# voletiv/mcvd-pytorch

Hardware: NVIDIA H100
Metric: frames/sec @100 DDPM steps, SMMNIST 64x64 (higher is better)
Workload: dtype f32 (fp16 hi/lo split on wgmma, fp32 accumulate)

## Files before the change

mcvd_b200/csrc/conv_umma.cu:

```cuda
#include <cuda.h>
#include <cuda_fp16.h>

#include <algorithm>
#include <cstring>

#include "mcvd_common.cuh"
#include "umma_ptx.cuh"

namespace mcvd {

constexpr int MT = 128;

namespace {

using namespace ptx;

constexpr int NPROD = 96;
constexpr int W_LOAD = 3;
constexpr int W_CONS = 4;
constexpr int NTHREADS = 384;
constexpr float STAT_SCALE = 65536.0f;
constexpr int TAB_NB = 8;
constexpr int HP_MAX = 512;
constexpr int PPT = (HP_MAX + NPROD - 1) / NPROD;
constexpr int RAW_STAGES = 2;
constexpr int MAX_RESIDENT = 12;

struct ConvMaps {
  CUtensorMap src[4];
  CUtensorMap tab;
};

struct ConvArgs {
  const float* s0;
  const float* s1;
  const float* s2;
  const float* s3;
  int C2, C3, nKB0;
  const __half* wpk;
  const float* bias;
  const float* res;
  const float* tab;
  int tab_planar;
  float* dst;
  unsigned long long* stats;
  int NJ;
  int B, H, W, C0, C1, Cout;
  int ks;
  int Wp, Pimg;
  int Qtot;
  int KB;
  int HP;
  int boxn, nbox;
  int raw_off, raw_stage, tab_off;
  int RA;
  int halo0;
  int nKB;
  int NB;
  int SA;
  int NPI;
  int tiles_n, ntiles;
  int act_in, act_out;
  int split;
  int tab_nb;
  float wscale, oscale;
};

__device__ __forceinline__ int decode_pos(const ConvArgs& a, int q, int& b_out) {
  if (q < 0 || q >= a.Qtot) return -1;
  const int b = q / a.Pimg;
  const int r = q - b * a.Pimg;
  const int rr = r / a.Wp, cc = r - rr * a.Wp;
  b_out = b;
  if (a.ks == 3) {
    if (rr == 0 || cc == 0) return -1;
    return (b * a.H + (rr - 1)) * a.W + (cc - 1);
  }
  return (b * a.H + rr) * a.W + cc;
}

__device__ __forceinline__ int first_raw(const ConvArgs& a, int q) {
  q = max(q, 0);
  if (q >= a.Qtot) return a.B * a.H * a.W;
  if (a.ks == 1) return q;
  const int b = q / a.Pimg;
  const int r = q - b * a.Pimg;
  const int rr = r / a.Wp, cc = r - rr * a.Wp;
  if (rr == 0) return b * a.H * a.W;
  return (b * a.H + (rr - 1)) * a.W + (cc == 0 ? 0 : cc - 1);
}

template <int NT>
__global__ void __launch_bounds__(NTHREADS, 1) k_conv_umma(const ConvArgs a, const __grid_constant__ ConvMaps maps) {
  extern __shared__ __align__(1024) uint8_t smem_raw[];
  const int chunks = a.KB / 8;
  const uint32_t a_half_bytes = (uint32_t)chunks * a.HP * 16;
  const uint32_t a_stage_bytes = 2 * a_half_bytes;
  constexpr uint32_t b_step_bytes = 64u * NT;
  const uint32_t b_stage_bytes = (uint32_t)(a.KB / 16) * b_step_bytes;
  uint8_t* a_base = smem_raw;
  uint8_t* b_base = a_base + (size_t)a.SA * a_stage_bytes;
  uint8_t* raw_base = smem_raw + a.raw_off;
  int* pinfo = reinterpret_cast<int*>(raw_base + (size_t)a.RA * a.raw_stage);
  unsigned long long* stat_s = reinterpret_cast<unsigned long long*>(pinfo + PPT * NPROD);
  uint64_t* bars = reinterpret_cast<uint64_t*>(stat_s + (a.stats ? a.NJ * 2 * NT : 0));
  const uint32_t bar0 = smem_u32(bars);
  auto A_FULL = [&](int i) { return bar0 + 8u * i; };
  auto A_EMPTY = [&](int i) { return bar0 + 8u * (a.SA + i); };
  auto B_FULL = [&](int i) { return bar0 + 8u * (2 * a.SA + i); };
  auto B_EMPTY = [&](int i) { return bar0 + 8u * (2 * a.SA + a.NB + i); };
  auto R_FULL = [&](int i) { return bar0 + 8u * (2 * a.SA + 2 * a.NB + i); };
  const int groups_n = a.tiles_n / a.NPI;

  const int tid = threadIdx.x, warp = tid >> 5, lane = tid & 31;
  const int taps = a.ks * a.ks;

  if (tid == 0) {
    for (int i = 0; i < a.SA; ++i) { mbar_init(A_FULL(i), NPROD); mbar_init(A_EMPTY(i), 8); }
    for (int i = 0; i < a.NB; ++i) { mbar_init(B_FULL(i), 1); mbar_init(B_EMPTY(i), 8); }
    for (int i = 0; i < a.RA; ++i) mbar_init(R_FULL(i), 1);
    fence_barrier_init();
  }
  if (a.stats)
    for (int i = tid; i < a.NJ * 2 * NT; i += NTHREADS) stat_s[i] = 0ull;
  __syncthreads();

  if (warp < W_LOAD) {
    const bool has_tab = a.tab != nullptr;
    const uint32_t rowb = (uint32_t)a.KB * 4, smask = a.KB == 32 ? 7u : 3u;
    auto tile_b0_of = [&](int t) {
      const int q_first = (t / groups_n) * MT - a.halo0;
      return q_first <= 0 ? 0 : min(a.B - 1, q_first / a.Pimg);
    };
    const uint32_t raw0 = smem_u32(raw_base);
    const uint32_t main_bytes = (uint32_t)a.nbox * a.boxn * rowb, ctr_bytes = (uint32_t)MT * rowb;
    const uint32_t tab_bytes = (uint32_t)a.tab_nb * a.KB * (a.tab_planar ? 12 : 16);
    int it = blockIdx.x, ikb = 0, ig = 0;
    auto issue_next = [&]() {
      if (it >= a.ntiles) return;
      const int p0 = (it / groups_n) * MT;
      const bool seg2 = ikb >= a.nKB0;
      int si, cc0;
      if (!seg2) {
        const int c0 = ikb * a.KB;
        if (c0 < a.C0) { si = 0; cc0 = c0; } else { si = 1; cc0 = c0 - a.C0; }
      } else {
        const int c0 = (ikb - a.nKB0) * a.KB;
        if (c0 < a.C2) { si = 2; cc0 = c0; } else { si = 3; cc0 = c0 - a.C2; }
      }
      const bool use_tab = has_tab && !seg2;
      const uint32_t dst = raw0 + (uint32_t)(ig % a.RA) * a.raw_stage;
      const uint32_t bar = R_FULL(ig % a.RA);
      mbar_arrive_expect_tx(bar, (seg2 ? ctr_bytes : main_bytes) + (use_tab ? tab_bytes : 0u));
      if (seg2) {
        tma_load_2d(dst, &maps.src[si], cc0, first_raw(a, p0), bar);
      } else {
        const int r0 = first_raw(a, p0 - a.halo0);
        for (int i = 0; i < a.nbox; ++i)
          tma_load_2d(dst + (uint32_t)i * a.boxn * rowb, &maps.src[si], cc0, r0 + i * a.boxn, bar);
      }
      if (use_tab) {
        if (a.tab_planar) tma_load_3d(dst + a.tab_off, &maps.tab, ikb * a.KB, 0, tile_b0_of(it), bar);
        else tma_load_2d(dst + a.tab_off, &maps.tab, 4 * ikb * a.KB, tile_b0_of(it), bar);
      }
      ++ig;
      if (++ikb == a.nKB) { ikb = 0; it += gridDim.x; }
    };
    if (tid == 0)
      for (int i = 0; i < a.RA - 1; ++i) issue_next();
    int g = 0;
    for (int t = blockIdx.x; t < a.ntiles; t += gridDim.x) {
      const int p0 = (t / groups_n) * MT;
      const int tb0 = tile_b0_of(t);
      const int raw_m = first_raw(a, p0 - a.halo0), raw_c = first_raw(a, p0);
      for (int h = tid; h < a.HP; h += NPROD) {
        int b = tb0;
        const int pix = decode_pos(a, p0 - a.halo0 + h, b);
        pinfo[h] = pix < 0 ? -1 : ((b - tb0) << 16) | (pix - raw_m);
      }
      for (int kb = 0; kb < a.nKB; ++kb, ++g) {
        const int st = g % a.SA;
        const bool seg2 = kb >= a.nKB0;
        const bool use_tab = has_tab && !seg2;
        const int h_lo = seg2 ? a.halo0 : 0, h_hi = seg2 ? a.halo0 + MT : a.HP;
        const int roff = seg2 ? raw_c - raw_m : 0;
        named_bar_sync(1, NPROD);
        if (tid == 0) issue_next();
        mbar_wait(A_EMPTY(st), ((g / a.SA) & 1) ^ 1);
        const int rs = g % a.RA;
        mbar_wait(R_FULL(rs), (g / a.RA) & 1);
        const uint8_t* raw = raw_base + (size_t)rs * a.raw_stage;
        const float* tsm = reinterpret_cast<const float*>(raw + a.tab_off);
        uint8_t* hi_base = a_base + (size_t)st * a_stage_bytes;
        uint8_t* lo_base = hi_base + a_half_bytes;
        const int h0 = h_lo + (tid - h_lo % NPROD + NPROD) % NPROD;
#pragma unroll 1
        for (int h = h0; h < h_hi; h += NPROD) {
          const int info = pinfo[h];
          const bool pad = info < 0;
          const int bidx = info >> 16;
          const uint32_t row = (uint32_t)((info & 0xffff) - roff);
          float4 rv[8];
#pragma unroll
          for (int j = 0; j < 8; ++j)
            if (j < 2 * chunks) {
              const uint32_t off = row * rowb + 16u * j;
              rv[j] = pad ? make_float4(0.f, 0.f, 0.f, 0.f)
                          : *reinterpret_cast<const float4*>(raw + (off ^ (((off >> 7) & smask) << 4)));
            }
#pragma unroll
          for (int ch = 0; ch < 4; ++ch) {
            if (ch < chunks) {
              uint4 hv = make_uint4(0u, 0u, 0u, 0u), lv = hv;
              if (!pad) {
                float v[8] = {rv[2 * ch].x, rv[2 * ch].y, rv[2 * ch].z, rv[2 * ch].w,
                              rv[2 * ch + 1].x, rv[2 * ch + 1].y, rv[2 * ch + 1].z, rv[2 * ch + 1].w};
                if (use_tab) {
                  if (a.tab_planar) {
                    const float* tb = tsm + bidx * 3 * a.KB + ch * 8;
#pragma unroll
                    for (int e = 0; e < 8; ++e) v[e] = fmaf(v[e] - tb[e], tb[a.KB + e], tb[2 * a.KB + e]);
                  } else {
                    const float4* tb = reinterpret_cast<const float4*>(tsm) + bidx * a.KB + ch * 8;
#pragma unroll
                    for (int e = 0; e < 8; ++e) {
                      const float4 tv = tb[e];
                      v[e] = fmaf(v[e] - tv.x, tv.y * tv.z, tv.w);
                    }
                  }
                  if (a.act_in) silu_fast8(v);
                }
                uint32_t hw[4], lw[4];
#pragma unroll
                for (int e = 0; e < 4; ++e) split2(v[2 * e], v[2 * e + 1], hw[e], lw[e]);
                hv = make_uint4(hw[0], hw[1], hw[2], hw[3]);
                lv = make_uint4(lw[0], lw[1], lw[2], lw[3]);
              }
              const size_t off = ((size_t)ch * a.HP + h) * 16;
              *reinterpret_cast<uint4*>(hi_base + off) = hv;
              *reinterpret_cast<uint4*>(lo_base + off) = lv;
            }
          }
        }
        fence_proxy_async();
        mbar_arrive(A_FULL(st));
      }
    }
  } else if (warp == W_LOAD) {
    if (elect_one()) {
      const uint32_t b0 = smem_u32(b_base);
      const int per_tile = a.nKB0 * taps + (a.nKB - a.nKB0);
      int st = 0, ph = 1;
      for (int t = blockIdx.x; t < a.ntiles; t += gridDim.x)
       for (int j = 0; j < a.NPI; ++j) {
        const int nt = (t % groups_n) * a.NPI + j;
        const uint8_t* wsrc = reinterpret_cast<const uint8_t*>(a.wpk) + (size_t)nt * per_tile * b_stage_bytes;
        for (int i = 0; i < per_tile; ++i) {
          mbar_wait(B_EMPTY(st), ph);
          mbar_arrive_expect_tx(B_FULL(st), b_stage_bytes);
          bulk_g2s(b0 + (uint32_t)st * b_stage_bytes, wsrc + (size_t)i * b_stage_bytes, b_stage_bytes, B_FULL(st));
          if (++st == a.NB) { st = 0; ph ^= 1; }
        }
      }
    }
    __syncwarp();
  } else {
    const int wg = (warp - W_CONS) >> 2;
    const int wq = (warp - W_CONS) & 3;
    const int ksteps = a.KB / 16;
    const uint32_t a_lbo = (uint32_t)a.HP * 16;
    const uint64_t a_proto = make_desc(0, a_lbo, 128), b_proto = make_desc(0, NT * 16, 128);
    const uint32_t a_half16 = a_half_bytes >> 4, b_lo16 = 2u * NT;
    const uint32_t a0_16 = smem_u32(a_base) >> 4, b0_16 = smem_u32(b_base) >> 4;
    const uint32_t a_stage16 = a_stage_bytes >> 4, b_stage16 = b_stage_bytes >> 4;
    const uint32_t a_lbo16 = a_lbo >> 4;
    int bst = 0, bph = 0, g0 = 0;
    for (int t = blockIdx.x; t < a.ntiles; t += gridDim.x, g0 += a.nKB)
     for (int j = 0; j < a.NPI; ++j) {
      const int p0 = (t / groups_n) * MT;
      const int n0 = ((t % groups_n) * a.NPI + j) * NT;
      const bool last_n = j == a.NPI - 1;
      float acc[NT / 2];
#pragma unroll
      for (int i = 0; i < NT / 2; ++i) acc[i] = 0.f;
      int pend_b = -1, pend_a = -1;
      for (int kb = 0; kb < a.nKB; ++kb) {
        const int g = g0 + kb;
        const int st = g % a.SA;
        mbar_wait(A_FULL(st), (g / a.SA) & 1);
        const uint32_t a_hi16 = a0_16 + (uint32_t)st * a_stage16 + (uint32_t)(a.halo0 + 64 * wg);
        const int ntap = (kb < a.nKB0) ? taps : 1;
        for (int tap = 0; tap < ntap; ++tap) {
          mbar_wait(B_FULL(bst), bph);
          const int shift = (a.ks == 3 && kb < a.nKB0) ? ((tap / 3 - 1) * a.Wp + (tap % 3 - 1)) : 0;
          const uint32_t a_tap16 = a_hi16 + (uint32_t)shift;
          const uint32_t b_tap16 = b0_16 + (uint32_t)bst * b_stage16;
          wgmma_fence();
#pragma unroll 1
          for (int s = 0; s < ksteps; ++s) {
            const uint64_t dbh = desc_add(b_proto, b_tap16 + (uint32_t)s * (b_step_bytes >> 4));
            const uint64_t dbl = desc_add(dbh, b_lo16);
            const uint64_t dah = desc_add(a_proto, a_tap16 + (uint32_t)(2 * s) * a_lbo16);
            const uint64_t dal = desc_add(dah, a_half16);
            wgmma_ss<NT>(acc, dah, dbh, 1);
            if (a.split & 1) wgmma_ss<NT>(acc, dal, dbh, 1);
            if (a.split & 2) wgmma_ss<NT>(acc, dah, dbl, 1);
          }
          wgmma_commit();
          wgmma_wait<1>();
          if (pend_b >= 0 && lane == 0) mbar_arrive(B_EMPTY(pend_b));
          if (pend_a >= 0 && lane == 0) mbar_arrive(A_EMPTY(pend_a));
          pend_b = bst;
          pend_a = (tap == ntap - 1 && last_n) ? st : -1;
          if (++bst == a.NB) { bst = 0; bph ^= 1; }
        }
      }
      wgmma_wait<0>();
#pragma unroll
      for (int i = 0; i < NT / 2; ++i) reg_fence(acc[i]);
      if (lane == 0) { mbar_arrive(B_EMPTY(pend_b)); if (pend_a >= 0) mbar_arrive(A_EMPTY(pend_a)); }

      const int r0 = 64 * wg + 16 * wq + (lane >> 2);
      const int cq = 2 * (lane & 3);
      int pix[2], slot[2];
      const int tile_b0 = min(a.B - 1, p0 / a.Pimg);
#pragma unroll
      for (int i = 0; i < 2; ++i) {
        int b = 0;
        pix[i] = decode_pos(a, p0 + r0 + 8 * i, b);
        slot[i] = pix[i] >= 0 ? b - tile_b0 : -1;
      }
      unsigned jmask = 0;
      if (a.stats) {
#pragma unroll 1
        for (int jj = 0; jj < a.NJ; ++jj)
          if (__ballot_sync(0xffffffffu, slot[0] == jj || slot[1] == jj)) jmask |= 1u << jj;
      }
#pragma unroll
      for (int j = 0; j < NT / 8; ++j) {
        const int n = n0 + 8 * j + cq;
        const float2 bv = a.bias ? __ldg(reinterpret_cast<const float2*>(a.bias + n)) : make_float2(0.f, 0.f);
        float v[2][2];
#pragma unroll
        for (int i = 0; i < 2; ++i) {
          float2 rv = make_float2(0.f, 0.f);
          if (a.res && pix[i] >= 0) rv = __ldg(reinterpret_cast<const float2*>(a.res + (long long)pix[i] * a.Cout + n));
          float x0 = (acc[4 * j + 2 * i] * a.wscale + bv.x + rv.x) * a.oscale;
          float x1 = (acc[4 * j + 2 * i + 1] * a.wscale + bv.y + rv.y) * a.oscale;
          if (a.act_out) { x0 = silu_f(x0); x1 = silu_f(x1); }
          v[i][0] = x0; v[i][1] = x1;
          if (pix[i] >= 0) *reinterpret_cast<float2*>(a.dst + (long long)pix[i] * a.Cout + n) = make_float2(x0, x1);
        }
        if (a.stats) {
#pragma unroll 1
          for (int jj = 0; jj < a.NJ; ++jj) {
            if (!(jmask & (1u << jj))) continue;
#pragma unroll
            for (int e = 0; e < 2; ++e) {
              long long s1 = 0;
              unsigned long long s2 = 0;
#pragma unroll
              for (int i = 0; i < 2; ++i) {
                if (slot[i] == jj) {
                  const int xi = __float2int_rn(v[i][e] * STAT_SCALE);
                  s1 += xi;
                  s2 += (unsigned long long)((long long)xi * (long long)xi);
                }
              }
#pragma unroll
              for (int o = 4; o <= 16; o <<= 1) {
                s1 += __shfl_xor_sync(0xffffffffu, s1, o);
                s2 += __shfl_xor_sync(0xffffffffu, s2, o);
              }
              if (lane < 4) {
                unsigned long long* sp = stat_s + (size_t)jj * 2 * NT + 8 * j + cq + e;
                atomicAdd(sp, (unsigned long long)s1);
                atomicAdd(sp + NT, s2);
              }
            }
          }
        }
      }
      if (a.stats) {
        named_bar_sync(2, 256);
        const int et = tid - W_CONS * 32;
        unsigned long long* gp = a.stats + (size_t)(p0 / MT) * a.NJ * 2 * a.Cout;
        for (int i = et; i < a.NJ * 2 * NT; i += 256) {
          const int jp = i / NT, n = i - jp * NT;
          gp[(size_t)jp * a.Cout + n0 + n] = stat_s[i];
          stat_s[i] = 0ull;
        }
        named_bar_sync(2, 256);
      }
    }
  }
}

__global__ void k_pack_weights(const float* __restrict__ w, __half* __restrict__ out, int taps, int Cin, int Cout,
                               int NT, int KB, float scale, int stage_off, int per_unit) {
  const int ksteps = KB / 16, nKB = Cin / KB, nNT = Cout / NT;
  const long long total = (long long)nNT * nKB * taps * ksteps * 2 * NT * 8;
  for (long long i = (long long)blockIdx.x * blockDim.x + threadIdx.x; i < total;
       i += (long long)gridDim.x * blockDim.x) {
    int e = (int)(i % 8);
    long long t = i / 8;
    int n = (int)(t % NT); t /= NT;
    int j = (int)(t % 2); t /= 2;
    int s = (int)(t % ksteps); t /= ksteps;
    int tap = (int)(t % taps); t /= taps;
    int kb = (int)(t % nKB); t /= nKB;
    int nt = (int)t;
    int c = kb * KB + s * 16 + j * 8 + e;
    float v = w[((long long)tap * Cin + c) * Cout + nt * NT + n] * scale;
    __half h = __float2half_rn(v);
    __half l = __float2half_rn(v - __half2float(h));
    long long step = ((long long)nt * per_unit + stage_off + (long long)kb * taps + tap) * ksteps + s;
    long long base = step * (4LL * NT * 8);
    long long o = (long long)(j * NT + n) * 8 + e;
    out[base + o] = h;
    out[base + 2LL * NT * 8 + o] = l;
  }
}

int pick_kb(int C0, int C1) {
  if (C0 % 32 == 0 && C1 % 32 == 0) return 32;
  if (C0 % 16 == 0 && C1 % 16 == 0) return 16;
  return 0;
}

int conv_kb(int C0, int C1, int C2, int C3) {
  int kb = pick_kb(C0, C1);
  if (C2 + C3 > 0 && pick_kb(C2, C3) < kb) kb = pick_kb(C2, C3);
  return kb;
}

struct Plan {
  int HP, NB, NJ;
  int boxn, nbox, tab_nb;
  int raw_off, raw_stage, tab_off, RA;
  size_t smem;
};

constexpr size_t SMEM_LIMIT = 227 * 1024;

size_t round1024(size_t x) { return (x + 1023) & ~(size_t)1023; }

bool make_plan(int H, int W, int ks, int KB, int NT, bool stats, int SA, Plan& p) {
  const int Wp = ks == 3 ? W + 1 : W;
  const int Pimg = ks == 3 ? (H + 1) * (W + 1) : H * W;
  const int halo0 = ks == 3 ? Wp + 1 : 0;
  p.HP = (MT + 2 * halo0 + 7) & ~7;
  p.NJ = (MT - 1) / Pimg + 2;
  if (p.HP > HP_MAX) return false;
  p.nbox = p.HP > 256 ? 2 : 1;
  p.boxn = p.nbox == 1 ? p.HP : ((p.HP / 2 + 7) & ~7);
  p.tab_nb = std::min(p.HP / Pimg + 2, TAB_NB);
  p.tab_off = p.nbox * p.boxn * KB * 4;
  p.raw_stage = (int)round1024((size_t)p.tab_off + (size_t)p.tab_nb * KB * 16);
  const size_t a_stage = (size_t)2 * (KB / 8) * p.HP * 16;
  const size_t b_stage = (size_t)(KB / 16) * 64 * NT;
  const size_t stat_bytes = stats ? (size_t)p.NJ * 2 * NT * 8 : 0;
  const size_t pinfo_bytes = (size_t)PPT * NPROD * 4;
  size_t bar_bytes = 0, fixed = 0;
  for (p.RA = RAW_STAGES; p.RA >= 1; --p.RA) {
    bar_bytes = 8 * (2 * SA + 20 + p.RA);
    fixed = round1024(SA * a_stage) + (size_t)p.RA * p.raw_stage + pinfo_bytes + stat_bytes + bar_bytes;
    if (fixed + 2 * b_stage <= SMEM_LIMIT) break;
  }
  if (p.RA == 0) return false;
  p.NB = (int)((SMEM_LIMIT - fixed) / b_stage);
  if (p.NB > 10) p.NB = 10;
  p.raw_off = (int)round1024(SA * a_stage + (size_t)p.NB * b_stage);
  p.smem = (size_t)p.raw_off + (size_t)p.RA * p.raw_stage + pinfo_bytes + stat_bytes + bar_bytes;
  return p.smem <= SMEM_LIMIT;
}

using EncodeTiled = CUresult (*)(CUtensorMap*, CUtensorMapDataType, cuuint32_t, void*, const cuuint64_t*,
                                 const cuuint64_t*, const cuuint32_t*, const cuuint32_t*, CUtensorMapInterleave,
                                 CUtensorMapSwizzle, CUtensorMapL2promotion, CUtensorMapFloatOOBfill);

EncodeTiled encode_tiled() {
  static const EncodeTiled fn = [] {
    void* f = nullptr;
    cudaDriverEntryPointQueryResult q;
    if (cudaGetDriverEntryPoint("cuTensorMapEncodeTiled", &f, cudaEnableDefault, &q) != cudaSuccess ||
        q != cudaDriverEntryPointSuccess)
      f = nullptr;
    return reinterpret_cast<EncodeTiled>(f);
  }();
  return fn;
}

int encode_map(CUtensorMap* m, const float* base, int rank, const cuuint64_t* dims, const cuuint64_t* strides,
               const cuuint32_t* box, CUtensorMapSwizzle swz, const char* name) {
  MCVD_CHECK(((uintptr_t)base & 15) == 0, "%s: TMA source %p is not 16-byte aligned", name, (const void*)base);
  for (int i = 0; i < rank; ++i)
    MCVD_CHECK(box[i] >= 1 && box[i] <= 256, "%s: TMA box dimension %u outside [1, 256]", name, box[i]);
  for (int i = 0; i < rank - 1; ++i)
    MCVD_CHECK(strides[i] % 16 == 0, "%s: TMA stride %llu bytes is not a multiple of 16", name,
               (unsigned long long)strides[i]);
  const EncodeTiled enc = encode_tiled();
  MCVD_CHECK(enc != nullptr, "%s: cuTensorMapEncodeTiled unavailable", name);
  const cuuint32_t estr[3] = {1, 1, 1};
  const CUresult r = enc(m, CU_TENSOR_MAP_DATA_TYPE_FLOAT32, (cuuint32_t)rank, const_cast<float*>(base), dims, strides,
                         box, estr, CU_TENSOR_MAP_INTERLEAVE_NONE, swz, CU_TENSOR_MAP_L2_PROMOTION_L2_128B,
                         CU_TENSOR_MAP_FLOAT_OOB_FILL_NONE);
  MCVD_CHECK(r == CUDA_SUCCESS, "%s: cuTensorMapEncodeTiled failed (%d)", name, (int)r);
  return 0;
}

template <int NT>
int launch_nt(const ConvArgs& a, const ConvMaps& m, size_t smem, int grid, cudaStream_t s) {
  cudaError_t e = cudaFuncSetAttribute(k_conv_umma<NT>, cudaFuncAttributeMaxDynamicSharedMemorySize, (int)smem);
  MCVD_CHECK(e == cudaSuccess, "CONV_UMMA: cudaFuncSetAttribute failed: %s", cudaGetErrorString(e));
  k_conv_umma<NT><<<grid, NTHREADS, smem, s>>>(a, m);
  MCVD_CUDA_LAUNCH_CHECK("conv_umma");
  return 0;
}

int launch_conv(const McvdOp& op, cudaStream_t s, bool planar) {
  const char* name = planar ? "CONV_UMMA2" : "CONV_UMMA";
  MCVD_CHECK(op.src0 && op.w && op.dst && (op.C1 == 0 || op.src1), "%s: null pointer", name);
  MCVD_CHECK(op.i0 == 1 || op.i0 == 3, "%s: kernel size %d unsupported", name, op.i0);
  ConvArgs a;
  a.s0 = (const float*)op.src0; a.s1 = (const float*)op.src1; a.wpk = (const __half*)op.w;
  a.s2 = (const float*)op.src2; a.s3 = (const float*)op.src3; a.C2 = op.src2 ? op.C2 : 0; a.C3 = op.src3 ? op.C3 : 0;
  a.bias = (const float*)op.bias; a.res = (const float*)op.aux0; a.tab = (const float*)op.aux1;
  a.tab_planar = planar ? 1 : 0;
  a.dst = (float*)op.dst;
  a.stats = (unsigned long long*)op.dst2;
  a.B = op.B; a.H = op.H; a.W = op.W; a.C0 = op.C0; a.C1 = op.C1; a.Cout = op.Cout; a.ks = op.i0;
  const int NT = op.i1;
  a.KB = conv_kb(op.C0, op.C1, a.C2, a.C3);
  MCVD_CHECK(a.KB != 0, "%s: input channels (%d,%d | %d,%d) must be multiples of 16", name, op.C0, op.C1, a.C2, a.C3);
  MCVD_CHECK(!planar || op.i2 == 0 || op.i2 == a.KB, "CONV_UMMA2: weights packed for K-block %d, the conv uses %d",
             op.i2, a.KB);
  MCVD_CHECK(NT >= 16 && NT <= 256 && NT % 16 == 0 && op.Cout % NT == 0, "%s: n tile %d invalid for Cout %d", name, NT,
             op.Cout);
  if (a.ks == 3) { a.Wp = op.W + 1; a.Pimg = (op.H + 1) * (op.W + 1); }
  else { a.Wp = op.W; a.Pimg = op.H * op.W; }
  MCVD_CHECK((long long)op.B * a.Pimg < (1LL << 31), "%s: too many pixels", name);
  a.Qtot = op.B * a.Pimg;
  MCVD_CHECK(!a.stats || a.Pimg >= 64, "%s: epilogue statistics need images of >= 64 positions", name);
  a.halo0 = (a.ks == 3) ? a.Wp + 1 : 0;
  a.nKB0 = (op.C0 + op.C1) / a.KB;
  a.nKB = a.nKB0 + (a.C2 + a.C3) / a.KB;
  a.tiles_n = op.Cout / NT;
  long long tiles_m = (a.Qtot + MT - 1) / MT;
  if (planar) tiles_m = (tiles_m + 1) & ~1LL;
  int dev = 0, sms = 132;
  cudaGetDevice(&dev);
  cudaDeviceGetAttribute(&sms, cudaDevAttrMultiProcessorCount, dev);
  const int mode = planar ? 0 : op.i2;
  MCVD_CHECK(mode >= 0 && mode <= 2, "%s: work organisation %d", name, mode);
  Plan p;
  const bool can_stay = a.ks == 1 && a.nKB == a.nKB0 && a.tiles_n > 1 && a.nKB <= MAX_RESIDENT &&
                        make_plan(op.H, op.W, a.ks, a.KB, NT, a.stats != nullptr, a.nKB, p);
  const bool stay = can_stay && (mode == 2 || (mode == 0 && 2 * tiles_m >= sms));
  a.SA = stay ? a.nKB : 2;
  a.NPI = stay ? a.tiles_n : 1;
  MCVD_CHECK(make_plan(op.H, op.W, a.ks, a.KB, NT, a.stats != nullptr, a.SA, p),
             "%s: tile does not fit shared memory (W=%d)", name, op.W);
  a.HP = p.HP; a.NB = p.NB; a.NJ = p.NJ;
  a.boxn = p.boxn; a.nbox = p.nbox; a.raw_off = p.raw_off; a.raw_stage = p.raw_stage; a.tab_off = p.tab_off;
  a.RA = p.RA;
  a.act_in = (op.flags & MCVD_F_ACT_IN) ? 1 : 0;
  a.act_out = (op.flags & MCVD_F_ACT_OUT) ? 1 : 0;
  a.wscale = op.f1; a.oscale = op.f0;
  a.split = (op.i3 >= 1 && op.i3 <= 3) ? op.i3 : (op.i3 == 4 ? 0 : 3);
  {
    const int nb = a.HP / a.Pimg + 2;
    MCVD_CHECK(nb <= TAB_NB || !a.tab, "%s: %dx%d images are too small for the fused-norm path", name, op.H, op.W);
    a.tab_nb = (nb <= TAB_NB) ? nb : 0;
  }
  ConvMaps maps;
  memset(&maps, 0, sizeof(maps));
  {
    const float* srcs[4] = {a.s0, a.s1, a.s2, a.s3};
    const int cs[4] = {a.C0, a.C1, a.C2, a.C3};
    const CUtensorMapSwizzle swz = a.KB == 32 ? CU_TENSOR_MAP_SWIZZLE_128B : CU_TENSOR_MAP_SWIZZLE_64B;
    for (int i = 0; i < 4; ++i) {
      if (!cs[i]) continue;
      MCVD_CHECK(srcs[i] != nullptr, "%s: null source %d", name, i);
      const cuuint64_t dims[2] = {(cuuint64_t)cs[i], (cuuint64_t)op.B * op.H * op.W};
      const cuuint64_t strides[1] = {(cuuint64_t)cs[i] * 4};
      const cuuint32_t box[2] = {(cuuint32_t)a.KB, (cuuint32_t)(i < 2 ? a.boxn : MT)};
      if (encode_map(&maps.src[i], srcs[i], 2, dims, strides, box, swz, name)) return -1;
    }
    if (a.tab) {
      const int Cin = op.C0 + op.C1;
      if (planar) {
        const cuuint64_t dims[3] = {(cuuint64_t)Cin, 3, (cuuint64_t)op.B};
        const cuuint64_t strides[2] = {(cuuint64_t)Cin * 4, (cuuint64_t)Cin * 12};
        const cuuint32_t box[3] = {(cuuint32_t)a.KB, 3, (cuuint32_t)a.tab_nb};
        if (encode_map(&maps.tab, a.tab, 3, dims, strides, box, CU_TENSOR_MAP_SWIZZLE_NONE, name)) return -1;
      } else {
        const cuuint64_t dims[2] = {(cuuint64_t)Cin * 4, (cuuint64_t)op.B};
        const cuuint64_t strides[1] = {(cuuint64_t)Cin * 16};
        const cuuint32_t box[2] = {(cuuint32_t)(4 * a.KB), (cuuint32_t)a.tab_nb};
        if (encode_map(&maps.tab, a.tab, 2, dims, strides, box, CU_TENSOR_MAP_SWIZZLE_NONE, name)) return -1;
      }
    }
  }
  MCVD_CHECK(tiles_m * a.tiles_n < (1LL << 31), "%s: too many tiles", name);
  a.ntiles = (int)(tiles_m * (a.tiles_n / a.NPI));
  const int grid = a.ntiles < sms ? a.ntiles : sms;
  switch (NT) {
#define MCVD_NT_CASE(n) case n: return launch_nt<n>(a, maps, p.smem, grid, s);
    MCVD_NT_CASE(16) MCVD_NT_CASE(32) MCVD_NT_CASE(48) MCVD_NT_CASE(64) MCVD_NT_CASE(80) MCVD_NT_CASE(96)
    MCVD_NT_CASE(112) MCVD_NT_CASE(128) MCVD_NT_CASE(144) MCVD_NT_CASE(160) MCVD_NT_CASE(176) MCVD_NT_CASE(192)
    MCVD_NT_CASE(208) MCVD_NT_CASE(224) MCVD_NT_CASE(240) MCVD_NT_CASE(256)
#undef MCVD_NT_CASE
    default: break;
  }
  MCVD_CHECK(false, "%s: n tile %d", name, NT);
}

long long pack(const float* w_taps, int taps, int Cin, int Cout, int n_tile, int KB, void* out, int scale_log2,
               int stage_off, int per_unit, void* stream) {
  if ((KB != 16 && KB != 32) || Cin % KB || n_tile < 16 || n_tile % 16 || Cout % n_tile) {
    set_error("umma_pack_weights: Cin %d / Cout %d / n_tile %d / KB %d unsupported", Cin, Cout, n_tile, KB);
    return -1;
  }
  const long long bytes = (long long)taps * Cin * Cout * 4;
  if (!out) return bytes;
  if (!w_taps) {
    set_error("umma_pack_weights: null input");
    return -1;
  }
  const float scale = ldexpf(1.0f, scale_log2);
  const long long total = (long long)taps * Cin * Cout;
  long long blocks = (total + 255) / 256;
  if (blocks > 132LL * 16) blocks = 132LL * 16;
  k_pack_weights<<<(unsigned)blocks, 256, 0, (cudaStream_t)stream>>>(w_taps, (__half*)out, taps, Cin, Cout, n_tile, KB,
                                                                      scale, stage_off, per_unit);
  if (cudaGetLastError() != cudaSuccess) {
    set_error("umma_pack_weights: launch failed");
    return -2;
  }
  return bytes;
}

}

int launch_conv_umma(const McvdOp& op, cudaStream_t s) { return launch_conv(op, s, false); }
int launch_conv_umma2(const McvdOp& op, cudaStream_t s) { return launch_conv(op, s, true); }

}

extern "C" int mcvd_umma_kblock(int C0, int C1) { return mcvd::pick_kb(C0, C1); }

extern "C" long long mcvd_umma_pack_weights(const float* w_taps, int taps, int Cin, int Cout, int n_tile, int KB,
                                            void* out, int scale_log2, void* stream) {
  return mcvd::pack(w_taps, taps, Cin, Cout, n_tile, KB, out, scale_log2, 0, KB ? (Cin / KB) * taps : 0, stream);
}

extern "C" int mcvd_umma2_plan(int H, int W, int ks, int C0, int C1, int C2, int C3, int n_tile, int stats) {
  const int kb = mcvd::conv_kb(C0, C1, C2, C3);
  mcvd::Plan p;
  if (!kb || n_tile < 16 || n_tile > 256 || n_tile % 16) return 0;
  return mcvd::make_plan(H, W, ks, kb, n_tile, stats != 0, 2, p) ? kb : 0;
}

extern "C" int mcvd_umma2_plan_info(int H, int W, int ks, int C0, int C1, int C2, int C3, int n_tile, int stats,
                                    int* out) {
  const int kb = mcvd_umma2_plan(H, W, ks, C0, C1, C2, C3, n_tile, stats);
  if (!kb || !out) return -1;
  mcvd::Plan p;
  mcvd::make_plan(H, W, ks, kb, n_tile, stats != 0, 2, p);
  out[0] = kb; out[1] = p.HP; out[2] = 2; out[3] = p.RA; out[4] = p.NB; out[5] = p.NJ; out[6] = 0;
  out[7] = (int)p.smem; out[8] = 1; out[9] = 1;
  return 0;
}

extern "C" long long mcvd_umma2_stats_bytes(int B, int H, int W, int ks, int Cout) {
  const long long pimg = ks == 3 ? (long long)(H + 1) * (W + 1) : (long long)H * W;
  const long long tiles = 2 * ((B * pimg + 2 * mcvd::MT - 1) / (2 * mcvd::MT));
  const long long nj = (mcvd::MT - 1) / pimg + 2;
  return tiles * nj * 2 * Cout * 8;
}

extern "C" long long mcvd_umma2_pack_weights(const float* w_taps, int taps, int Cin, int Cout, int n_tile, int KB,
                                             void* out, int scale_log2, int stage_off, int per_unit, void* stream) {
  return mcvd::pack(w_taps, taps, Cin, Cout, n_tile, KB, out, scale_log2, stage_off, per_unit, stream);
}
```

mcvd_b200/csrc/umma_ptx.cuh:

```cuda
#pragma once
#include <cuda_fp16.h>
#include <stdint.h>

#include "wgmma_ops.cuh"

namespace mcvd {
namespace ptx {

__device__ __forceinline__ uint32_t smem_u32(const void* p) { return (uint32_t)__cvta_generic_to_shared(p); }

__device__ __forceinline__ void mbar_init(uint32_t bar, uint32_t count) {
  asm volatile("mbarrier.init.shared::cta.b64 [%0], %1;" ::"r"(bar), "r"(count) : "memory");
}
__device__ __forceinline__ void mbar_arrive(uint32_t bar) {
  asm volatile("{\n\t.reg .b64 st;\n\tmbarrier.arrive.shared::cta.b64 st, [%0];\n\t}" ::"r"(bar) : "memory");
}
__device__ __forceinline__ void mbar_arrive_expect_tx(uint32_t bar, uint32_t bytes) {
  asm volatile("{\n\t.reg .b64 st;\n\tmbarrier.arrive.expect_tx.shared::cta.b64 st, [%0], %1;\n\t}" ::"r"(bar),
               "r"(bytes)
               : "memory");
}
__device__ __forceinline__ void mbar_wait(uint32_t bar, uint32_t parity) {
  uint32_t done;
  do {
    asm volatile(
        "{\n\t"
        ".reg .pred p;\n\t"
        "mbarrier.try_wait.parity.shared::cta.b64 p, [%1], %2;\n\t"
        "selp.u32 %0, 1, 0, p;\n\t"
        "}"
        : "=r"(done)
        : "r"(bar), "r"(parity)
        : "memory");
  } while (!done);
}
__device__ __forceinline__ void named_bar_sync(int id, int nthreads) {
  asm volatile("bar.sync %0, %1;" ::"r"(id), "r"(nthreads) : "memory");
}
__device__ __forceinline__ void bulk_g2s(uint32_t dst, const void* src, uint32_t bytes, uint32_t bar) {
  asm volatile("cp.async.bulk.shared::cluster.global.mbarrier::complete_tx::bytes [%0], [%1], %2, [%3];" ::"r"(dst),
               "l"(src), "r"(bytes), "r"(bar)
               : "memory");
}
__device__ __forceinline__ void tma_load_2d(uint32_t dst, const void* map, int c0, int c1, uint32_t bar) {
  asm volatile(
      "cp.async.bulk.tensor.2d.shared::cluster.global.tile.mbarrier::complete_tx::bytes [%0], [%1, {%2, %3}], [%4];" ::"r"(
          dst),
      "l"(map), "r"(c0), "r"(c1), "r"(bar)
      : "memory");
}
__device__ __forceinline__ void tma_load_3d(uint32_t dst, const void* map, int c0, int c1, int c2, uint32_t bar) {
  asm volatile(
      "cp.async.bulk.tensor.3d.shared::cluster.global.tile.mbarrier::complete_tx::bytes [%0], [%1, {%2, %3, %4}], [%5];" ::"r"(
          dst),
      "l"(map), "r"(c0), "r"(c1), "r"(c2), "r"(bar)
      : "memory");
}
__device__ __forceinline__ void fence_proxy_async() { asm volatile("fence.proxy.async.shared::cta;" ::: "memory"); }
__device__ __forceinline__ void fence_barrier_init() { asm volatile("fence.mbarrier_init.release.cluster;" ::: "memory"); }

__device__ __forceinline__ void wgmma_fence() { asm volatile("wgmma.fence.sync.aligned;" ::: "memory"); }
__device__ __forceinline__ void wgmma_commit() { asm volatile("wgmma.commit_group.sync.aligned;" ::: "memory"); }
template <int N>
__device__ __forceinline__ void wgmma_wait() {
  asm volatile("wgmma.wait_group.sync.aligned %0;" ::"n"(N) : "memory");
}
__device__ __forceinline__ void reg_fence(float& r) { asm volatile("" : "+f"(r)::"memory"); }

__device__ __forceinline__ uint64_t make_desc(uint32_t saddr, uint32_t lbo_bytes, uint32_t sbo_bytes) {
  uint64_t d = 0;
  d |= (uint64_t)((saddr >> 4) & 0x3FFFu);
  d |= (uint64_t)((lbo_bytes >> 4) & 0x3FFFu) << 16;
  d |= (uint64_t)((sbo_bytes >> 4) & 0x3FFFu) << 32;
  return d;
}
__device__ __forceinline__ uint64_t desc_add(uint64_t d, uint32_t units16) { return d + (uint64_t)units16; }

__device__ __forceinline__ uint32_t pack_half2(__half a, __half b) {
  return (uint32_t)__half_as_ushort(a) | ((uint32_t)__half_as_ushort(b) << 16);
}

__device__ __forceinline__ bool elect_one() {
  uint32_t pred;
  asm volatile(
      "{\n\t"
      ".reg .pred p;\n\t"
      "elect.sync _|p, 0xffffffff;\n\t"
      "selp.u32 %0, 1, 0, p;\n\t"
      "}"
      : "=r"(pred));
  return pred != 0;
}

__device__ __forceinline__ float silu_fast(float x) {
  float e, r;
  asm("ex2.approx.ftz.f32 %0, %1;" : "=f"(e) : "f"(x * -1.4426950408889634f));
  asm("rcp.approx.ftz.f32 %0, %1;" : "=f"(r) : "f"(1.0f + e));
  return x * r;
}
__device__ __forceinline__ void silu_fast8(float v[8]) {
  float t[8];
#pragma unroll
  for (int e = 0; e < 8; ++e) t[e] = v[e] * -1.4426950408889634f;
#pragma unroll
  for (int e = 0; e < 8; ++e) asm volatile("ex2.approx.ftz.f32 %0, %0;" : "+f"(t[e]));
#pragma unroll
  for (int e = 0; e < 8; ++e) t[e] += 1.0f;
#pragma unroll
  for (int e = 0; e < 8; ++e) asm volatile("rcp.approx.ftz.f32 %0, %0;" : "+f"(t[e]));
#pragma unroll
  for (int e = 0; e < 8; ++e) v[e] *= t[e];
}
__device__ __forceinline__ void split2(float a, float b, uint32_t& hi, uint32_t& lo) {
  asm("cvt.rn.satfinite.f16x2.f32 %0, %1, %2;" : "=r"(hi) : "f"(b), "f"(a));
  const float2 hf = __half22float2(*reinterpret_cast<const __half2*>(&hi));
  asm("cvt.rn.satfinite.f16x2.f32 %0, %1, %2;" : "=r"(lo) : "f"(b - hf.y), "f"(a - hf.x));
}

}
}
```

Baseline: 119.5.

## Add 192-row M tiles with three consumer warpgroups and register reallocation

Templates the wgmma conv kernel on the number of consumer warpgroups so a tile can cover 192 output positions with three consumer warpgroups instead of 128 with two. It uses setmaxnreg to move registers from the producer warpgroup to the consumers. The host heuristic picks 192-row tiles when streaming, without stats or planar tables, when enough B stages fit and the last-wave imbalance does not grow. The aim is more reuse of the B weights per load and fewer tiles. The cost is more shared memory per stage and register pressure limits, and the wider tile only applies to eligible layers.

```diff
diff --git a/mcvd_b200/csrc/conv_umma.cu b/mcvd_b200/csrc/conv_umma.cu
--- a/mcvd_b200/csrc/conv_umma.cu
+++ b/mcvd_b200/csrc/conv_umma.cu
@@ -9,7 +9,7 @@
 
 namespace mcvd {
 
-constexpr int MT = 128;
+constexpr int STAT_MT = 128;
 
 namespace {
 
@@ -18,7 +18,8 @@
 constexpr int NPROD = 96;
 constexpr int W_LOAD = 3;
 constexpr int W_CONS = 4;
-constexpr int NTHREADS = 384;
+constexpr int NT_MAX3 = 192;
+constexpr int REG_PROD3 = 96, REG_CONS3 = 136;
 constexpr float STAT_SCALE = 65536.0f;
 constexpr int TAB_NB = 8;
 constexpr int HP_MAX = 512;
@@ -90,8 +91,13 @@
   return (b * a.H + (rr - 1)) * a.W + (cc == 0 ? 0 : cc - 1);
 }
 
-template <int NT>
-__global__ void __launch_bounds__(NTHREADS, 1) k_conv_umma(const ConvArgs a, const __grid_constant__ ConvMaps maps) {
+template <int NT, int NWG>
+__global__ void __launch_bounds__(128 * (NWG + 1), 1) k_conv_umma(const ConvArgs a,
+                                                                  const __grid_constant__ ConvMaps maps) {
+  static_assert(NWG == 2 || (NWG == 3 && NT <= NT_MAX3), "three consumer warpgroups hold at most 96 accumulators");
+  constexpr int MT = 64 * NWG;
+  constexpr int NTHREADS = 128 * (NWG + 1);
+  constexpr int NCONS = 4 * NWG;
   extern __shared__ __align__(1024) uint8_t smem_raw[];
   const int chunks = a.KB / 8;
   const uint32_t a_half_bytes = (uint32_t)chunks * a.HP * 16;
@@ -116,8 +122,8 @@
   const int taps = a.ks * a.ks;
 
   if (tid == 0) {
-    for (int i = 0; i < a.SA; ++i) { mbar_init(A_FULL(i), NPROD); mbar_init(A_EMPTY(i), 8); }
-    for (int i = 0; i < a.NB; ++i) { mbar_init(B_FULL(i), 1); mbar_init(B_EMPTY(i), 8); }
+    for (int i = 0; i < a.SA; ++i) { mbar_init(A_FULL(i), NPROD); mbar_init(A_EMPTY(i), NCONS); }
+    for (int i = 0; i < a.NB; ++i) { mbar_init(B_FULL(i), 1); mbar_init(B_EMPTY(i), NCONS); }
     for (int i = 0; i < a.RA; ++i) mbar_init(R_FULL(i), 1);
     fence_barrier_init();
   }
@@ -125,146 +131,150 @@
     for (int i = tid; i < a.NJ * 2 * NT; i += NTHREADS) stat_s[i] = 0ull;
   __syncthreads();
 
-  if (warp < W_LOAD) {
-    const bool has_tab = a.tab != nullptr;
-    const uint32_t rowb = (uint32_t)a.KB * 4, smask = a.KB == 32 ? 7u : 3u;
-    auto tile_b0_of = [&](int t) {
-      const int q_first = (t / groups_n) * MT - a.halo0;
-      return q_first <= 0 ? 0 : min(a.B - 1, q_first / a.Pimg);
-    };
-    const uint32_t raw0 = smem_u32(raw_base);
-    const uint32_t main_bytes = (uint32_t)a.nbox * a.boxn * rowb, ctr_bytes = (uint32_t)MT * rowb;
-    const uint32_t tab_bytes = (uint32_t)a.tab_nb * a.KB * (a.tab_planar ? 12 : 16);
-    int it = blockIdx.x, ikb = 0, ig = 0;
-    auto issue_next = [&]() {
-      if (it >= a.ntiles) return;
-      const int p0 = (it / groups_n) * MT;
-      const bool seg2 = ikb >= a.nKB0;
-      int si, cc0;
-      if (!seg2) {
-        const int c0 = ikb * a.KB;
-        if (c0 < a.C0) { si = 0; cc0 = c0; } else { si = 1; cc0 = c0 - a.C0; }
-      } else {
-        const int c0 = (ikb - a.nKB0) * a.KB;
-        if (c0 < a.C2) { si = 2; cc0 = c0; } else { si = 3; cc0 = c0 - a.C2; }
-      }
-      const bool use_tab = has_tab && !seg2;
-      const uint32_t dst = raw0 + (uint32_t)(ig % a.RA) * a.raw_stage;
-      const uint32_t bar = R_FULL(ig % a.RA);
-      mbar_arrive_expect_tx(bar, (seg2 ? ctr_bytes : main_bytes) + (use_tab ? tab_bytes : 0u));
-      if (seg2) {
-        tma_load_2d(dst, &maps.src[si], cc0, first_raw(a, p0), bar);
-      } else {
-        const int r0 = first_raw(a, p0 - a.halo0);
-        for (int i = 0; i < a.nbox; ++i)
-          tma_load_2d(dst + (uint32_t)i * a.boxn * rowb, &maps.src[si], cc0, r0 + i * a.boxn, bar);
-      }
-      if (use_tab) {
-        if (a.tab_planar) tma_load_3d(dst + a.tab_off, &maps.tab, ikb * a.KB, 0, tile_b0_of(it), bar);
-        else tma_load_2d(dst + a.tab_off, &maps.tab, 4 * ikb * a.KB, tile_b0_of(it), bar);
-      }
-      ++ig;
-      if (++ikb == a.nKB) { ikb = 0; it += gridDim.x; }
-    };
-    if (tid == 0)
-      for (int i = 0; i < a.RA - 1; ++i) issue_next();
-    int g = 0;
-    for (int t = blockIdx.x; t < a.ntiles; t += gridDim.x) {
-      const int p0 = (t / groups_n) * MT;
-      const int tb0 = tile_b0_of(t);
-      const int raw_m = first_raw(a, p0 - a.halo0), raw_c = first_raw(a, p0);
-      for (int h = tid; h < a.HP; h += NPROD) {
-        int b = tb0;
-        const int pix = decode_pos(a, p0 - a.halo0 + h, b);
-        pinfo[h] = pix < 0 ? -1 : ((b - tb0) << 16) | (pix - raw_m);
-      }
-      for (int kb = 0; kb < a.nKB; ++kb, ++g) {
-        const int st = g % a.SA;
-        const bool seg2 = kb >= a.nKB0;
+  if (warp < W_CONS) {
+    if constexpr (NWG == 3) setmaxnreg_dec<REG_PROD3>();
+    if (warp < W_LOAD) {
+      const bool has_tab = a.tab != nullptr;
+      const uint32_t rowb = (uint32_t)a.KB * 4, smask = a.KB == 32 ? 7u : 3u;
+      auto tile_b0_of = [&](int t) {
+        const int q_first = (t / groups_n) * MT - a.halo0;
+        return q_first <= 0 ? 0 : min(a.B - 1, q_first / a.Pimg);
+      };
+      const uint32_t raw0 = smem_u32(raw_base);
+      const uint32_t main_bytes = (uint32_t)a.nbox * a.boxn * rowb, ctr_bytes = (uint32_t)MT * rowb;
+      const uint32_t tab_bytes = (uint32_t)a.tab_nb * a.KB * (a.tab_planar ? 12 : 16);
+      int it = blockIdx.x, ikb = 0, ig = 0;
+      auto issue_next = [&]() {
+        if (it >= a.ntiles) return;
+        const int p0 = (it / groups_n) * MT;
+        const bool seg2 = ikb >= a.nKB0;
+        int si, cc0;
+        if (!seg2) {
+          const int c0 = ikb * a.KB;
+          if (c0 < a.C0) { si = 0; cc0 = c0; } else { si = 1; cc0 = c0 - a.C0; }
+        } else {
+          const int c0 = (ikb - a.nKB0) * a.KB;
+          if (c0 < a.C2) { si = 2; cc0 = c0; } else { si = 3; cc0 = c0 - a.C2; }
+        }
         const bool use_tab = has_tab && !seg2;
-        const int h_lo = seg2 ? a.halo0 : 0, h_hi = seg2 ? a.halo0 + MT : a.HP;
-        const int roff = seg2 ? raw_c - raw_m : 0;
-        named_bar_sync(1, NPROD);
-        if (tid == 0) issue_next();
-        mbar_wait(A_EMPTY(st), ((g / a.SA) & 1) ^ 1);
-        const int rs = g % a.RA;
-        mbar_wait(R_FULL(rs), (g / a.RA) & 1);
-        const uint8_t* raw = raw_base + (size_t)rs * a.raw_stage;
-        const float* tsm = reinterpret_cast<const float*>(raw + a.tab_off);
-        uint8_t* hi_base = a_base + (size_t)st * a_stage_bytes;
-        uint8_t* lo_base = hi_base + a_half_bytes;
-        const int h0 = h_lo + (tid - h_lo % NPROD + NPROD) % NPROD;
+        const uint32_t dst = raw0 + (uint32_t)(ig % a.RA) * a.raw_stage;
+        const uint32_t bar = R_FULL(ig % a.RA);
+        mbar_arrive_expect_tx(bar, (seg2 ? ctr_bytes : main_bytes) + (use_tab ? tab_bytes : 0u));
+        if (seg2) {
+          tma_load_2d(dst, &maps.src[si], cc0, first_raw(a, p0), bar);
+        } else {
+          const int r0 = first_raw(a, p0 - a.halo0);
+          for (int i = 0; i < a.nbox; ++i)
+            tma_load_2d(dst + (uint32_t)i * a.boxn * rowb, &maps.src[si], cc0, r0 + i * a.boxn, bar);
+        }
+        if (use_tab) {
+          if (a.tab_planar) tma_load_3d(dst + a.tab_off, &maps.tab, ikb * a.KB, 0, tile_b0_of(it), bar);
+          else tma_load_2d(dst + a.tab_off, &maps.tab, 4 * ikb * a.KB, tile_b0_of(it), bar);
+        }
+        ++ig;
+        if (++ikb == a.nKB) { ikb = 0; it += gridDim.x; }
+      };
+      if (tid == 0)
+        for (int i = 0; i < a.RA - 1; ++i) issue_next();
+      int g = 0;
+      for (int t = blockIdx.x; t < a.ntiles; t += gridDim.x) {
+        const int p0 = (t / groups_n) * MT;
+        const int tb0 = tile_b0_of(t);
+        const int raw_m = first_raw(a, p0 - a.halo0), raw_c = first_raw(a, p0);
+        for (int h = tid; h < a.HP; h += NPROD) {
+          int b = tb0;
+          const int pix = decode_pos(a, p0 - a.halo0 + h, b);
+          pinfo[h] = pix < 0 ? -1 : ((b - tb0) << 16) | (pix - raw_m);
+        }
+        for (int kb = 0; kb < a.nKB; ++kb, ++g) {
+          const int st = g % a.SA;
+          const bool seg2 = kb >= a.nKB0;
+          const bool use_tab = has_tab && !seg2;
+          const int h_lo = seg2 ? a.halo0 : 0, h_hi = seg2 ? a.halo0 + MT : a.HP;
+          const int roff = seg2 ? raw_c - raw_m : 0;
+          named_bar_sync(1, NPROD);
+          if (tid == 0) issue_next();
+          mbar_wait(A_EMPTY(st), ((g / a.SA) & 1) ^ 1);
+          const int rs = g % a.RA;
+          mbar_wait(R_FULL(rs), (g / a.RA) & 1);
+          const uint8_t* raw = raw_base + (size_t)rs * a.raw_stage;
+          const float* tsm = reinterpret_cast<const float*>(raw + a.tab_off);
+          uint8_t* hi_base = a_base + (size_t)st * a_stage_bytes;
+          uint8_t* lo_base = hi_base + a_half_bytes;
+          const int h0 = h_lo + (tid - h_lo % NPROD + NPROD) % NPROD;
 #pragma unroll 1
-        for (int h = h0; h < h_hi; h += NPROD) {
-          const int info = pinfo[h];
-          const bool pad = info < 0;
-          const int bidx = info >> 16;
-          const uint32_t row = (uint32_t)((info & 0xffff) - roff);
-          float4 rv[8];
-#pragma unroll
-          for (int j = 0; j < 8; ++j)
-            if (j < 2 * chunks) {
-              const uint32_t off = row * rowb + 16u * j;
-              rv[j] = pad ? make_float4(0.f, 0.f, 0.f, 0.f)
-                          : *reinterpret_cast<const float4*>(raw + (off ^ (((off >> 7) & smask) << 4)));
-            }
-#pragma unroll
-          for (int ch = 0; ch < 4; ++ch) {
-            if (ch < chunks) {
-              uint4 hv = make_uint4(0u, 0u, 0u, 0u), lv = hv;
-              if (!pad) {
-                float v[8] = {rv[2 * ch].x, rv[2 * ch].y, rv[2 * ch].z, rv[2 * ch].w,
-                              rv[2 * ch + 1].x, rv[2 * ch + 1].y, rv[2 * ch + 1].z, rv[2 * ch + 1].w};
-                if (use_tab) {
-                  if (a.tab_planar) {
-                    const float* tb = tsm + bidx * 3 * a.KB + ch * 8;
-#pragma unroll
-                    for (int e = 0; e < 8; ++e) v[e] = fmaf(v[e] - tb[e], tb[a.KB + e], tb[2 * a.KB + e]);
-                  } else {
-                    const float4* tb = reinterpret_cast<const float4*>(tsm) + bidx * a.KB + ch * 8;
-#pragma unroll
-                    for (int e = 0; e < 8; ++e) {
-                      const float4 tv = tb[e];
-                      v[e] = fmaf(v[e] - tv.x, tv.y * tv.z, tv.w);
+          for (int h = h0; h < h_hi; h += NPROD) {
+            const int info = pinfo[h];
+            const bool pad = info < 0;
+            const int bidx = info >> 16;
+            const uint32_t row = (uint32_t)((info & 0xffff) - roff);
+            float4 rv[8];
+#pragma unroll
+            for (int j = 0; j < 8; ++j)
+              if (j < 2 * chunks) {
+                const uint32_t off = row * rowb + 16u * j;
+                rv[j] = pad ? make_float4(0.f, 0.f, 0.f, 0.f)
+                            : *reinterpret_cast<const float4*>(raw + (off ^ (((off >> 7) & smask) << 4)));
+              }
+#pragma unroll
+            for (int ch = 0; ch < 4; ++ch) {
+              if (ch < chunks) {
+                uint4 hv = make_uint4(0u, 0u, 0u, 0u), lv = hv;
+                if (!pad) {
+                  float v[8] = {rv[2 * ch].x, rv[2 * ch].y, rv[2 * ch].z, rv[2 * ch].w,
+                                rv[2 * ch + 1].x, rv[2 * ch + 1].y, rv[2 * ch + 1].z, rv[2 * ch + 1].w};
+                  if (use_tab) {
+                    if (a.tab_planar) {
+                      const float* tb = tsm + bidx * 3 * a.KB + ch * 8;
+#pragma unroll
+                      for (int e = 0; e < 8; ++e) v[e] = fmaf(v[e] - tb[e], tb[a.KB + e], tb[2 * a.KB + e]);
+                    } else {
+                      const float4* tb = reinterpret_cast<const float4*>(tsm) + bidx * a.KB + ch * 8;
+#pragma unroll
+                      for (int e = 0; e < 8; ++e) {
+                        const float4 tv = tb[e];
+                        v[e] = fmaf(v[e] - tv.x, tv.y * tv.z, tv.w);
+                      }
                     }
+                    if (a.act_in) silu_fast8(v);
                   }
-                  if (a.act_in) silu_fast8(v);
+                  uint32_t hw[4], lw[4];
+#pragma unroll
+                  for (int e = 0; e < 4; ++e) split2(v[2 * e], v[2 * e + 1], hw[e], lw[e]);
+                  hv = make_uint4(hw[0], hw[1], hw[2], hw[3]);
+                  lv = make_uint4(lw[0], lw[1], lw[2], lw[3]);
                 }
-                uint32_t hw[4], lw[4];
-#pragma unroll
-                for (int e = 0; e < 4; ++e) split2(v[2 * e], v[2 * e + 1], hw[e], lw[e]);
-                hv = make_uint4(hw[0], hw[1], hw[2], hw[3]);
-                lv = make_uint4(lw[0], lw[1], lw[2], lw[3]);
+                const size_t off = ((size_t)ch * a.HP + h) * 16;
+                *reinterpret_cast<uint4*>(hi_base + off) = hv;
+                *reinterpret_cast<uint4*>(lo_base + off) = lv;
               }
-              const size_t off = ((size_t)ch * a.HP + h) * 16;
-              *reinterpret_cast<uint4*>(hi_base + off) = hv;
-              *reinterpret_cast<uint4*>(lo_base + off) = lv;
             }
           }
-        }
-        fence_proxy_async();
-        mbar_arrive(A_FULL(st));
+          fence_proxy_async();
+          mbar_arrive(A_FULL(st));
+        }
       }
+    } else if (warp == W_LOAD) {
+      if (elect_one()) {
+        const uint32_t b0 = smem_u32(b_base);
+        const int per_tile = a.nKB0 * taps + (a.nKB - a.nKB0);
+        int st = 0, ph = 1;
+        for (int t = blockIdx.x; t < a.ntiles; t += gridDim.x)
+         for (int j = 0; j < a.NPI; ++j) {
+          const int nt = (t % groups_n) * a.NPI + j;
+          const uint8_t* wsrc = reinterpret_cast<const uint8_t*>(a.wpk) + (size_t)nt * per_tile * b_stage_bytes;
+          for (int i = 0; i < per_tile; ++i) {
+            mbar_wait(B_EMPTY(st), ph);
+            mbar_arrive_expect_tx(B_FULL(st), b_stage_bytes);
+            bulk_g2s(b0 + (uint32_t)st * b_stage_bytes, wsrc + (size_t)i * b_stage_bytes, b_stage_bytes, B_FULL(st));
+            if (++st == a.NB) { st = 0; ph ^= 1; }
+          }
+        }
+      }
+      __syncwarp();
     }
-  } else if (warp == W_LOAD) {
-    if (elect_one()) {
-      const uint32_t b0 = smem_u32(b_base);
-      const int per_tile = a.nKB0 * taps + (a.nKB - a.nKB0);
-      int st = 0, ph = 1;
-      for (int t = blockIdx.x; t < a.ntiles; t += gridDim.x)
-       for (int j = 0; j < a.NPI; ++j) {
-        const int nt = (t % groups_n) * a.NPI + j;
-        const uint8_t* wsrc = reinterpret_cast<const uint8_t*>(a.wpk) + (size_t)nt * per_tile * b_stage_bytes;
-        for (int i = 0; i < per_tile; ++i) {
-          mbar_wait(B_EMPTY(st), ph);
-          mbar_arrive_expect_tx(B_FULL(st), b_stage_bytes);
-          bulk_g2s(b0 + (uint32_t)st * b_stage_bytes, wsrc + (size_t)i * b_stage_bytes, b_stage_bytes, B_FULL(st));
-          if (++st == a.NB) { st = 0; ph ^= 1; }
-        }
-      }
-    }
-    __syncwarp();
   } else {
+    if constexpr (NWG == 3) setmaxnreg_inc<REG_CONS3>();
     const int wg = (warp - W_CONS) >> 2;
     const int wq = (warp - W_CONS) & 3;
     const int ksteps = a.KB / 16;
@@ -382,15 +392,15 @@
         }
       }
       if (a.stats) {
-        named_bar_sync(2, 256);
+        named_bar_sync(2, 32 * NCONS);
         const int et = tid - W_CONS * 32;
         unsigned long long* gp = a.stats + (size_t)(p0 / MT) * a.NJ * 2 * a.Cout;
-        for (int i = et; i < a.NJ * 2 * NT; i += 256) {
+        for (int i = et; i < a.NJ * 2 * NT; i += 32 * NCONS) {
           const int jp = i / NT, n = i - jp * NT;
           gp[(size_t)jp * a.Cout + n0 + n] = stat_s[i];
           stat_s[i] = 0ull;
         }
-        named_bar_sync(2, 256);
+        named_bar_sync(2, 32 * NCONS);
       }
     }
   }
@@ -445,7 +455,7 @@
 
 size_t round1024(size_t x) { return (x + 1023) & ~(size_t)1023; }
 
-bool make_plan(int H, int W, int ks, int KB, int NT, bool stats, int SA, Plan& p) {
+bool make_plan(int H, int W, int ks, int KB, int NT, bool stats, int SA, int MT, Plan& p) {
   const int Wp = ks == 3 ? W + 1 : W;
   const int Pimg = ks == 3 ? (H + 1) * (W + 1) : H * W;
   const int halo0 = ks == 3 ? Wp + 1 : 0;
@@ -509,13 +519,20 @@
   return 0;
 }
 
-template <int NT>
+template <int NT, int NWG>
 int launch_nt(const ConvArgs& a, const ConvMaps& m, size_t smem, int grid, cudaStream_t s) {
-  cudaError_t e = cudaFuncSetAttribute(k_conv_umma<NT>, cudaFuncAttributeMaxDynamicSharedMemorySize, (int)smem);
+  cudaError_t e = cudaFuncSetAttribute(k_conv_umma<NT, NWG>, cudaFuncAttributeMaxDynamicSharedMemorySize, (int)smem);
   MCVD_CHECK(e == cudaSuccess, "CONV_UMMA: cudaFuncSetAttribute failed: %s", cudaGetErrorString(e));
-  k_conv_umma<NT><<<grid, NTHREADS, smem, s>>>(a, m);
+  k_conv_umma<NT, NWG><<<grid, 128 * (NWG + 1), smem, s>>>(a, m);
   MCVD_CUDA_LAUNCH_CHECK("conv_umma");
   return 0;
+}
+
+template <int NT>
+int launch_nt(const ConvArgs& a, const ConvMaps& m, size_t smem, int grid, int nwg, cudaStream_t s) {
+  if constexpr (NT <= NT_MAX3)
+    if (nwg == 3) return launch_nt<NT, 3>(a, m, smem, grid, s);
+  return launch_nt<NT, 2>(a, m, smem, grid, s);
 }
 
 int launch_conv(const McvdOp& op, cudaStream_t s, bool planar) {
@@ -546,8 +563,7 @@
   a.nKB0 = (op.C0 + op.C1) / a.KB;
   a.nKB = a.nKB0 + (a.C2 + a.C3) / a.KB;
   a.tiles_n = op.Cout / NT;
-  long long tiles_m = (a.Qtot + MT - 1) / MT;
-  if (planar) tiles_m = (tiles_m + 1) & ~1LL;
+  const long long tiles128 = (a.Qtot + STAT_MT - 1) / STAT_MT;
   int dev = 0, sms = 132;
   cudaGetDevice(&dev);
   cudaDeviceGetAttribute(&sms, cudaDevAttrMultiProcessorCount, dev);
@@ -555,11 +571,27 @@
   MCVD_CHECK(mode >= 0 && mode <= 2, "%s: work organisation %d", name, mode);
   Plan p;
   const bool can_stay = a.ks == 1 && a.nKB == a.nKB0 && a.tiles_n > 1 && a.nKB <= MAX_RESIDENT &&
-                        make_plan(op.H, op.W, a.ks, a.KB, NT, a.stats != nullptr, a.nKB, p);
-  const bool stay = can_stay && (mode == 2 || (mode == 0 && 2 * tiles_m >= sms));
+                        make_plan(op.H, op.W, a.ks, a.KB, NT, a.stats != nullptr, a.nKB, STAT_MT, p);
+  const bool stay = can_stay && (mode == 2 || (mode == 0 && 2 * tiles128 >= sms));
   a.SA = stay ? a.nKB : 2;
   a.NPI = stay ? a.tiles_n : 1;
-  MCVD_CHECK(make_plan(op.H, op.W, a.ks, a.KB, NT, a.stats != nullptr, a.SA, p),
+  const int mt_req = planar ? 0 : op.i4;
+  MCVD_CHECK(mt_req == 0 || mt_req == 128 || mt_req == 192, "%s: tile height %d", name, mt_req);
+  const bool can3 = !planar && NT <= NT_MAX3 && !stay && !a.stats &&
+                    make_plan(op.H, op.W, a.ks, a.KB, NT, false, a.SA, 192, p) &&
+                    (!a.tab || p.HP / a.Pimg + 2 <= TAB_NB);
+  MCVD_CHECK(mt_req != 192 || can3, "%s: 192-position tiles need streaming, NT <= %d, no statistics and %dx%d to fit",
+             name, NT_MAX3, op.H, op.W);
+  auto last_positions = [&](int mt) {
+    const long long items = (a.Qtot + mt - 1) / mt * a.tiles_n;
+    return (items + sms - 1) / sms * mt;
+  };
+  const bool wide_slab = a.ks == 3 && op.W >= 64 && a.nKB == a.nKB0;
+  const int MT = mt_req ? mt_req
+                        : (can3 && p.NB >= 3 && !wide_slab && last_positions(192) <= last_positions(128) ? 192 : 128);
+  long long tiles_m = (a.Qtot + MT - 1) / MT;
+  if (planar) tiles_m = (tiles_m + 1) & ~1LL;
+  MCVD_CHECK(make_plan(op.H, op.W, a.ks, a.KB, NT, a.stats != nullptr, a.SA, MT, p),
              "%s: tile does not fit shared memory (W=%d)", name, op.W);
   a.HP = p.HP; a.NB = p.NB; a.NJ = p.NJ;
   a.boxn = p.boxn; a.nbox = p.nbox; a.raw_off = p.raw_off; a.raw_stage = p.raw_stage; a.tab_off = p.tab_off;
@@ -606,7 +638,7 @@
   a.ntiles = (int)(tiles_m * (a.tiles_n / a.NPI));
   const int grid = a.ntiles < sms ? a.ntiles : sms;
   switch (NT) {
-#define MCVD_NT_CASE(n) case n: return launch_nt<n>(a, maps, p.smem, grid, s);
+#define MCVD_NT_CASE(n) case n: return launch_nt<n>(a, maps, p.smem, grid, MT / 64, s);
     MCVD_NT_CASE(16) MCVD_NT_CASE(32) MCVD_NT_CASE(48) MCVD_NT_CASE(64) MCVD_NT_CASE(80) MCVD_NT_CASE(96)
     MCVD_NT_CASE(112) MCVD_NT_CASE(128) MCVD_NT_CASE(144) MCVD_NT_CASE(160) MCVD_NT_CASE(176) MCVD_NT_CASE(192)
     MCVD_NT_CASE(208) MCVD_NT_CASE(224) MCVD_NT_CASE(240) MCVD_NT_CASE(256)
@@ -659,7 +691,7 @@
   const int kb = mcvd::conv_kb(C0, C1, C2, C3);
   mcvd::Plan p;
   if (!kb || n_tile < 16 || n_tile > 256 || n_tile % 16) return 0;
-  return mcvd::make_plan(H, W, ks, kb, n_tile, stats != 0, 2, p) ? kb : 0;
+  return mcvd::make_plan(H, W, ks, kb, n_tile, stats != 0, 2, mcvd::STAT_MT, p) ? kb : 0;
 }
 
 extern "C" int mcvd_umma2_plan_info(int H, int W, int ks, int C0, int C1, int C2, int C3, int n_tile, int stats,
@@ -667,7 +699,7 @@
   const int kb = mcvd_umma2_plan(H, W, ks, C0, C1, C2, C3, n_tile, stats);
   if (!kb || !out) return -1;
   mcvd::Plan p;
-  mcvd::make_plan(H, W, ks, kb, n_tile, stats != 0, 2, p);
+  mcvd::make_plan(H, W, ks, kb, n_tile, stats != 0, 2, mcvd::STAT_MT, p);
   out[0] = kb; out[1] = p.HP; out[2] = 2; out[3] = p.RA; out[4] = p.NB; out[5] = p.NJ; out[6] = 0;
   out[7] = (int)p.smem; out[8] = 1; out[9] = 1;
   return 0;
@@ -675,8 +707,8 @@
 
 extern "C" long long mcvd_umma2_stats_bytes(int B, int H, int W, int ks, int Cout) {
   const long long pimg = ks == 3 ? (long long)(H + 1) * (W + 1) : (long long)H * W;
-  const long long tiles = 2 * ((B * pimg + 2 * mcvd::MT - 1) / (2 * mcvd::MT));
-  const long long nj = (mcvd::MT - 1) / pimg + 2;
+  const long long tiles = 2 * ((B * pimg + 2 * mcvd::STAT_MT - 1) / (2 * mcvd::STAT_MT));
+  const long long nj = (mcvd::STAT_MT - 1) / pimg + 2;
   return tiles * nj * 2 * Cout * 8;
 }
 
diff --git a/mcvd_b200/csrc/umma_ptx.cuh b/mcvd_b200/csrc/umma_ptx.cuh
--- a/mcvd_b200/csrc/umma_ptx.cuh
+++ b/mcvd_b200/csrc/umma_ptx.cuh
@@ -56,6 +56,10 @@
       "l"(map), "r"(c0), "r"(c1), "r"(c2), "r"(bar)
       : "memory");
 }
+template <int R>
+__device__ __forceinline__ void setmaxnreg_dec() { asm volatile("setmaxnreg.dec.sync.aligned.u32 %0;" ::"n"(R)); }
+template <int R>
+__device__ __forceinline__ void setmaxnreg_inc() { asm volatile("setmaxnreg.inc.sync.aligned.u32 %0;" ::"n"(R)); }
 __device__ __forceinline__ void fence_proxy_async() { asm volatile("fence.proxy.async.shared::cta;" ::: "memory"); }
 __device__ __forceinline__ void fence_barrier_init() { asm volatile("fence.mbarrier_init.release.cluster;" ::: "memory"); }
 
```

New measurement: 126.9 (median of 6 runs). 1.06x the previous value.
